# huawei-noah/xingtian

Hardware: NVIDIA H100
Metric: learner env-steps/sec (Atari 84x84x4 PPO) (higher is better)
Workload: dtype f32 (bf16x3 split on wgmma, fp32 accumulate in registers)

## Files before the change

xingtian_b200/csrc/bp_gemm.cuh:

```cuda
#pragma once
#include <cuda_bf16.h>
#include <cuda_runtime.h>
#include <stdint.h>

#include "gemm_f32.cuh"

#ifndef XTB_BP_WAIT_HINT
#define XTB_BP_WAIT_HINT 20000u
#endif

namespace xtb {
namespace bp {

typedef __nv_bfloat16 bf16;

__device__ __forceinline__ uint32_t smem_u32(const void* p) { return (uint32_t)__cvta_generic_to_shared(p); }
__device__ __forceinline__ void mbar_init(uint32_t bar, uint32_t count) {
  asm volatile("mbarrier.init.shared::cta.b64 [%0], %1;" ::"r"(bar), "r"(count) : "memory");
}
__device__ __forceinline__ void fence_barrier_init() { asm volatile("fence.mbarrier_init.release.cluster;" ::: "memory"); }
__device__ __forceinline__ void mbar_arrive(uint32_t bar) {
  asm volatile("mbarrier.arrive.shared::cta.b64 _, [%0];" ::"r"(bar) : "memory");
}
__device__ __forceinline__ void mbar_expect_tx(uint32_t bar, uint32_t bytes) {
// ... 180 lines not shown
  split2(v[6], v[7], hi.w, lo.w);
}

struct BpT {
  bf16* hi;
  long long lo_off;
  int pitch;
};
__host__ __device__ inline long long bp_index(int pitch, int row, int f) { return ((long long)(f >> 3) * pitch + row) * 8 + (f & 7); }

constexpr int BP_CONSUMER_WGS = 2;
constexpr int BP_P_WARP = 4 * BP_CONSUMER_WGS;
constexpr int BP_THREADS = 32 * (BP_P_WARP + 1);
constexpr int BP_CONSUMER_WARPS = 4 * BP_CONSUMER_WGS;

constexpr int RW_THREADS = BP_THREADS;
constexpr int RW_A_PLANE = 2048;
constexpr int RW_STAGE_A = 2 * 8 * RW_A_PLANE;
constexpr int RW_STAGE_B = 16384;
constexpr int RW_MAX_STAGES = 4;
constexpr int RW_EPI_BANKS = 2;

__host__ __device__ inline int dgrad_epi_planes(int src_act, int accumulate) {
  return (src_act == 1 ? 1 : (src_act == 2 ? 2 : 0)) + (accumulate ? 2 : 0);
}

struct StageEnt {
  uint32_t a_chunk;
  uint16_t w_row;
  uint16_t nch;
};
typedef uint32_t UnitEnt;
struct StageDesc { uint32_t a_off, w_off, nch; };

struct RowsArgs {
  BpT a; int a_split;
  const bf16* w_hi; const bf16* w_lo; int w_pitch;
  int w_res; int w_res_chunks;
  int mode;
  const StageEnt* stages; const UnitEnt* units;
  int n_stage_ents;
  int kchunks, kc_split, n_ntiles;
  int n_units, n_btiles, B, N;
  BpT out; float* out_f32; int ld_f32; const float* bias; float alpha; int act;
  float* part; long long part_z; int ld_part;
  BpT src; int src_act; int accumulate; float* db_part;
};

struct TileWalk {
  const uint2* stages_sm; const uint32_t* units_sm;
  uint32_t a_pstride, w_pitch; int mode, n_ntiles, kc_split, kchunks, N;
  const uint2* st; uint32_t a0, w0, da, dw; int ns, nch_last;
  __device__ __forceinline__ void setup(const RowsArgs& a, const uint2* s_sm, const uint32_t* u_sm) {
    stages_sm = s_sm; units_sm = u_sm;
    a_pstride = (uint32_t)a.a.pitch * 16u; w_pitch = (uint32_t)a.w_pitch;
    mode = a.mode; n_ntiles = a.n_ntiles; kc_split = a.kc_split; kchunks = a.kchunks; N = a.N;
  }
  template <int KIND>
// ... 11 lines not shown
      const uint32_t ue = units_sm[u];
      st = stages_sm + (ue & 0xffffffu); ns = (int)(ue >> 24);
    }
  }
  __device__ __forceinline__ StageDesc get(int s) const {
    if (st) {
      const uint2 v = st[s];
      return StageDesc{v.x * a_pstride, (v.y & 0xffffu) * 16u, v.y >> 16};
    }
    return StageDesc{a0 + (uint32_t)s * da, w0 + (uint32_t)s * dw, (uint32_t)(s == ns - 1 ? nch_last : 8)};
  }
};

template <int KIND, int N>
__global__ void __launch_bounds__(RW_THREADS, 1)
bp_rows_kernel(const __grid_constant__ RowsArgs a, int n_stages, int stage_bytes, int wres_bytes, int epi_banks) {
  extern __shared__ uint8_t smem_raw[];
  uint8_t* smem = reinterpret_cast<uint8_t*>((reinterpret_cast<uintptr_t>(smem_raw) + 127) & ~(uintptr_t)127);
  constexpr int NCH = N >> 3;
  const int epi_planes = KIND == 2 ? dgrad_epi_planes(a.src_act, a.accumulate) : 0;
  const int epi_bank_bytes = epi_planes * NCH * RW_A_PLANE;
  uint8_t* epi_sm = smem + wres_bytes + n_stages * stage_bytes;
  uint2* stages_sm = reinterpret_cast<uint2*>(epi_sm + epi_banks * epi_bank_bytes);
  uint32_t* units_sm = reinterpret_cast<uint32_t*>(stages_sm + a.n_stage_ents);
  __shared__ __align__(8) uint64_t bars[2 * RW_MAX_STAGES + 1 + 2 * RW_EPI_BANKS];
  __shared__ float red_sh[BP_CONSUMER_WARPS][64];
  __shared__ float bias_sh[64];

  const int tid = threadIdx.x, warp = __shfl_sync(0xffffffffu, tid >> 5, 0), lane = tid & 31;
  const uint32_t full0 = smem_u32(&bars[0]), empty0 = smem_u32(&bars[RW_MAX_STAGES]), wbar = smem_u32(&bars[2 * RW_MAX_STAGES]);
  const uint32_t efull0 = wbar + 8, eempty0 = efull0 + 8 * RW_EPI_BANKS;
  if (tid == 0) {
    for (int s = 0; s < RW_MAX_STAGES; s++) { mbar_init(full0 + 8 * s, 1); mbar_init(empty0 + 8 * s, BP_CONSUMER_WARPS); }
    mbar_init(wbar, 1);
    for (int k = 0; k < RW_EPI_BANKS; k++) { mbar_init(efull0 + 8 * k, 1); mbar_init(eempty0 + 8 * k, BP_CONSUMER_WARPS); }
    fence_barrier_init();
  }
  __syncthreads();
  if (a.mode != 2) {
    const uint2* gs = reinterpret_cast<const uint2*>(a.stages);
    for (int i = tid; i < a.n_stage_ents; i += RW_THREADS) stages_sm[i] = __ldg(gs + i);
    for (int i = tid; i < a.n_units; i += RW_THREADS) units_sm[i] = __ldg(a.units + i);
  }
  if (warp == BP_P_WARP && a.w_res && elect_one()) {
    const uint32_t bytes = (uint32_t)a.w_res_chunks * a.w_pitch * 16;
    mbar_expect_tx(wbar, 2 * bytes);
    bulk_g2s(smem_u32(smem), a.w_hi, bytes, wbar);
    bulk_g2s(smem_u32(smem) + bytes, a.w_lo, bytes, wbar);
  }
  pdl_wait();
  pdl_trigger();
  if (KIND == 0 && a.mode != 2 && tid < N) bias_sh[tid] = a.bias[tid];
  __syncthreads();
  const uint32_t wres = smem_u32(smem);
  const uint32_t stage0 = wres + (uint32_t)wres_bytes;
  const int total = a.n_units * a.n_btiles;
  constexpr bool CAT = (KIND != 2);
  const int nbt = a.n_btiles;
  const int du = (int)gridDim.x / nbt, dbt = (int)gridDim.x - du * nbt;

  if (warp == BP_P_WARP) {
    const bool a_split = a.a_split != 0, w_res = a.w_res != 0;
    const uint32_t a_pstride = (uint32_t)a.a.pitch * 16u, w_pstride = (uint32_t)a.w_pitch * 16u;
    const char* a_hi = reinterpret_cast<const char*>(a.a.hi);
    const char* a_lo = a_hi + a.a.lo_off * 2;
    const char* w_hi = reinterpret_cast<const char*>(a.w_hi);
    const char* w_lo = reinterpret_cast<const char*>(a.w_lo);
    constexpr int n_bh_fwd = N >> 3;
    int stage = 0; uint32_t phase = 0;
    int u = (int)blockIdx.x / nbt, bt = (int)blockIdx.x - u * nbt;
    const int Bsz = a.B;
    TileWalk tw; tw.setup(a, stages_sm, units_sm);
    const int src_act = a.src_act, accumulate = a.accumulate;
    const char* s_hi = reinterpret_cast<const char*>(a.src.hi);
    const char* s_lo = s_hi + a.src.lo_off * 2;
    const char* o_hi = reinterpret_cast<const char*>(a.out.hi);
    const char* o_lo = o_hi + a.out.lo_off * 2;
    const uint32_t s_ps = (uint32_t)a.src.pitch * 16u, o_ps = (uint32_t)a.out.pitch * 16u;
    int ebank = 0; uint32_t ephase = 0;
    for (int tile = blockIdx.x; tile < total; tile += gridDim.x) {
      const int b0 = bt * 128, nr = min(128, Bsz - b0);
      const uint32_t a_bytes = (uint32_t)nr * 16u, row_off = (uint32_t)b0 * 16u;
      tw.init<KIND>(u);
      for (int s = 0; s < tw.ns; s++) {
        const StageDesc d = tw.get(s);
        mbar_wait(empty0 + 8 * stage, phase ^ 1);
        const int nch = (int)d.nch;
        const int n_bh = w_res ? 0 : (KIND == 2 ? nch : n_bh_fwd);
        const uint32_t b_bytes = (KIND == 2) ? (uint32_t)N * 16u : (uint32_t)nch * 128u;
        const uint32_t fb = full0 + 8 * stage;
        if (elect_one()) {
          mbar_expect_tx(fb, a_bytes * (a_split ? 2 * nch : nch) + b_bytes * 2 * n_bh);
          const uint32_t sA = stage0 + (uint32_t)stage * stage_bytes, sB = sA + RW_STAGE_A;
          const char* ah = a_hi + d.a_off + row_off;
          for (int c = 0; c < nch; c++) bulk_g2s(sA + c * RW_A_PLANE, ah + (uint32_t)c * a_pstride, a_bytes, fb);
          if (a_split) {
            const char* al = a_lo + d.a_off + row_off;
            for (int c = 0; c < nch; c++) bulk_g2s(sA + 8 * RW_A_PLANE + c * RW_A_PLANE, al + (uint32_t)c * a_pstride, a_bytes, fb);
          }
          if (!w_res) {
            const char* wh = w_hi + d.w_off; const char* wl = w_lo + d.w_off;
            if (KIND == 2) {
              for (int c = 0; c < n_bh; c++) {
                bulk_g2s(sB + c * (N * 16), wh + (uint32_t)c * w_pstride, b_bytes, fb);
                bulk_g2s(sB + 8192 + c * (N * 16), wl + (uint32_t)c * w_pstride, b_bytes, fb);
              }
            } else {
              for (int c = 0; c < n_bh; c++) {
                bulk_g2s(sB + c * 1024, wh + (uint32_t)c * w_pstride, b_bytes, fb);
                bulk_g2s(sB + (n_bh_fwd + c) * 1024, wl + (uint32_t)c * w_pstride, b_bytes, fb);
              }
            }
          }
        }
        __syncwarp();
        if (++stage == n_stages) { stage = 0; phase ^= 1; }
      }
      if (KIND == 2 && epi_planes) {
        mbar_wait(eempty0 + 8 * ebank, ephase ^ 1);
        if (elect_one()) {
          const uint32_t fb = efull0 + 8 * ebank;
          mbar_expect_tx(fb, a_bytes * (uint32_t)(NCH * epi_planes));
          const uint32_t oc0 = (uint32_t)((tw.mode == 2 ? u % tw.n_ntiles : u) * NCH);
          uint32_t dst = smem_u32(epi_sm) + (uint32_t)(ebank * epi_bank_bytes);
          auto plane = [&](const char* base, uint32_t ps) {
            const char* src = base + oc0 * ps + row_off;
            for (int c = 0; c < NCH; c++, dst += RW_A_PLANE) bulk_g2s(dst, src + (uint32_t)c * ps, a_bytes, fb);
          };
          if (src_act == 1 || src_act == 2) plane(s_hi, s_ps);
          if (src_act == 2) plane(s_lo, s_ps);
          if (accumulate) { plane(o_hi, o_ps); plane(o_lo, o_ps); }
        }
        __syncwarp();
        if (++ebank == epi_banks) { ebank = 0; ephase ^= 1; }
      }
      u += du; bt += dbt;
      if (bt >= nbt) { bt -= nbt; u++; }
    }
  } else if (warp < BP_P_WARP) {
    constexpr int ACC = CAT ? 2 * N : N;
    float dbacc[N / 4];
#pragma unroll
    for (int j = 0; j < N / 4; j++) dbacc[j] = 0.f;
    const int wg = warp >> 2, q = lane & 3;
    const int row_in_tile = wg * 64 + (warp & 3) * 16 + (lane >> 2);
    const bool a_split = a.a_split != 0, w_res = a.w_res != 0;
    const int act = a.act, mode = a.mode, Bsz = a.B, n_nt = a.n_ntiles, ld_f32 = a.ld_f32, src_act = a.src_act, accumulate = a.accumulate;
    const int ld_part = a.ld_part;
    const float alpha = a.alpha;
    bf16* const out_hi = a.out.hi; const long long out_lo = a.out.lo_off;
    float* const out_f32 = a.out_f32; const float* const bias_g = a.bias;
    float* const part = a.part; const long long part_z = a.part_z;
    const long long out_pstride = (long long)a.out.pitch * 8;
    const int b_pad = (Bsz + 15) & ~15;
    const uint32_t epi_thr = smem_u32(epi_sm) + (uint32_t)(row_in_tile * 16 + 4 * q);
    const int epi_out_plane = epi_planes - (accumulate ? 2 : 0);
    int ebank = 0; uint32_t ephase = 0;
    const uint64_t adesc = make_desc(0, RW_A_PLANE, 128);
    const uint64_t bdesc = (KIND == 2) ? make_desc(0, (uint32_t)N * 16, 128) : make_desc(0, 128, 1024);
    const uint32_t a_row_add = (uint32_t)(wg * 64 * 16) >> 4;
    const uint32_t a_lo_add = (8 * RW_A_PLANE) >> 4, a_step = (2 * RW_A_PLANE) >> 4;
    const uint32_t w_pstride = (uint32_t)a.w_pitch * 16u;
    const uint64_t wdesc = (KIND == 2) ? make_desc(0, w_pstride, 128) : make_desc(0, 128, w_pstride);
    const uint32_t w_lo_add = ((uint32_t)a.w_res_chunks * w_pstride) >> 4;
    const uint32_t b_step = (KIND == 2) ? (w_res ? (2 * w_pstride) >> 4 : (2u * N * 16u) >> 4) : (256 >> 4);
    const uint32_t b_lo_add = w_res ? w_lo_add : (8192 >> 4);
    const uint64_t b_const = w_res ? wdesc : bdesc;
    if (w_res) mbar_wait(wbar, 0);
    int stage = 0; uint32_t phase = 0;
    int held = -1;
    auto idle = [&](int bt) { return bt * 128 + wg * 64 >= Bsz; };

    auto mma_stage = [&](float* acc, const StageDesc& d, bool first, bool skip) {
      mbar_wait(full0 + 8 * stage, phase);
      const uint32_t sA = stage0 + (uint32_t)stage * stage_bytes;
      uint32_t a_lo32 = (sA >> 4) + a_row_add;
      uint32_t b_lo32 = w_res ? (wres + d.w_off) >> 4 : (sA + RW_STAGE_A) >> 4;
      const int ksteps = __shfl_sync(0xffffffffu, skip ? 0 : (int)d.nch >> 1, 0);
      uint32_t sd = first ? 0u : 1u;
      wgmma_fence();
      if (a_split) {
        for (int j = 0; j < ksteps; j++) {
          const uint64_t ah = adesc | a_lo32, bh = b_const | b_lo32, al = adesc | (a_lo32 + a_lo_add);
          if (KIND != 2) {
            wgmma<2 * N, 0, 1>(acc, ah, bh, sd);
            wgmma<N, 0, 1>(acc, al, bh);
          } else {
            wgmma<N, 0, 0>(acc, ah, bh, sd);
            wgmma<N, 0, 0>(acc, ah, b_const | (b_lo32 + b_lo_add));
            wgmma<N, 0, 0>(acc, al, bh);
          }
          a_lo32 += a_step; b_lo32 += b_step; sd = 1u;
        }
      } else {
        for (int j = 0; j < ksteps; j++) {
          const uint64_t ah = adesc | a_lo32, bh = b_const | b_lo32;
          if (KIND != 2) {
            wgmma<2 * N, 0, 1>(acc, ah, bh, sd);
          } else {
            wgmma<N, 0, 0>(acc, ah, bh, sd);
            wgmma<N, 0, 0>(acc, ah, b_const | (b_lo32 + b_lo_add));
          }
          a_lo32 += a_step; b_lo32 += b_step; sd = 1u;
        }
      }
      wgmma_commit();
      wgmma_wait<1>();
      if (held >= 0 && lane == 0) mbar_arrive(empty0 + 8 * held);
      held = stage;
      if (++stage == n_stages) { stage = 0; phase ^= 1; }
    };

    int tile = blockIdx.x;
    int u = (int)blockIdx.x / nbt, bt = (int)blockIdx.x - u * nbt;
    TileWalk tw; tw.setup(a, stages_sm, units_sm);
    auto start_tile = [&](float* acc) {
      tw.init<KIND>(u);
      tw.ns = __shfl_sync(0xffffffffu, tw.ns, 0);
      if (tw.ns == 0) return false;
      discard_regs<ACC / 2>(acc);
      mma_stage(acc, tw.get(0), true, idle(bt));
      return true;
    };

    auto epilogue = [&](const float* cur, int cu, int cbt, bool empty, uint32_t eb) {
      const int btile0 = cbt * 128;
      int oc0, z = 0;
      if (mode == 2) { const int nt = cu % n_nt; z = cu / n_nt; oc0 = nt * NCH; }
      else oc0 = cu * NCH;
#pragma unroll
      for (int h = 0; h < 2; h++) {
        const int b = btile0 + row_in_tile + 8 * h;
#pragma unroll
        for (int i = 0; i < NCH; i++) {
          const int c = 8 * i + 2 * q;
          float v0 = cur[4 * i + 2 * h], v1 = cur[4 * i + 2 * h + 1];
          if (CAT) { v0 += cur[4 * (i + NCH) + 2 * h]; v1 += cur[4 * (i + NCH) + 2 * h + 1]; }
          if (empty) { v0 = 0.f; v1 = 0.f; }
          if (KIND == 0) {
            if (b < Bsz) {
              const int f = oc0 * 8 + c;
              float bb0, bb1;
              if (mode == 2) { const float2 t2 = __ldg(reinterpret_cast<const float2*>(bias_g + f)); bb0 = t2.x; bb1 = t2.y; }
              else { bb0 = bias_sh[c]; bb1 = bias_sh[c + 1]; }
              if (act == 2) { v0 = tanhf(alpha * v0 + bb0); v1 = tanhf(alpha * v1 + bb1); }
              else {
                const float lo = act == 1 ? 0.f : -INFINITY;
// ... 2 lines not shown
              if (out_hi) {
                bf16* p = out_hi + (long long)(oc0 + i) * out_pstride + (long long)b * 8 + 2 * q;
                uint32_t hi, lo;
                split2(v0, v1, hi, lo);
                *reinterpret_cast<uint32_t*>(p) = hi;
                *reinterpret_cast<uint32_t*>(p + out_lo) = lo;
              }
              if (out_f32) *reinterpret_cast<float2*>(out_f32 + (long long)b * ld_f32 + f) = make_float2(v0, v1);
            }
          } else if (KIND == 1) {
            if (b < Bsz)
              *reinterpret_cast<float2*>(part + (long long)z * part_z + (long long)b * ld_part + oc0 * 8 + c) = make_float2(v0, v1);
          } else {
            bf16* p = out_hi + (long long)(oc0 + i) * out_pstride + (long long)b * 8 + 2 * q;
            if (b < Bsz) {
              const uint32_t e = eb + (uint32_t)(i * RW_A_PLANE + 128 * h);
              if (src_act == 1) {
                float s0, s1;
                unpack2(lds_u32(e), s0, s1);
                v0 = s0 > 0.f ? v0 : 0.f; v1 = s1 > 0.f ? v1 : 0.f;
              } else if (src_act == 2) {
                float s0, s1, t0, t1;
                unpack2(lds_u32(e), s0, s1);
                unpack2(lds_u32(e + NCH * RW_A_PLANE), t0, t1);
                const float y0 = s0 + t0, y1 = s1 + t1;
                v0 *= 1.f - y0 * y0; v1 *= 1.f - y1 * y1;
              }
              dbacc[2 * i] += v0; dbacc[2 * i + 1] += v1;
              if (accumulate) {
                const uint32_t eo = e + (uint32_t)(epi_out_plane * NCH * RW_A_PLANE);
                float s0, s1, t0, t1;
                unpack2(lds_u32(eo), s0, s1);
                unpack2(lds_u32(eo + NCH * RW_A_PLANE), t0, t1);
                v0 += s0 + t0; v1 += s1 + t1;
              }
              uint32_t hi, lo;
              split2(v0, v1, hi, lo);
              *reinterpret_cast<uint32_t*>(p) = hi;
              *reinterpret_cast<uint32_t*>(p + out_lo) = lo;
            } else if (b < b_pad && !accumulate) {
              *reinterpret_cast<uint32_t*>(p) = 0u;
              *reinterpret_cast<uint32_t*>(p + out_lo) = 0u;
            }
          }
        }
      }
    };

    constexpr bool OVERLAP = !(KIND == 0 && N == 64);
    auto finish_tile = [&](float* cur, float* nxt) {
      for (int s = 1; s < tw.ns; s++) mma_stage(cur, tw.get(s), false, idle(bt));
      const bool empty = tw.ns == 0;
      const int cu = u, cbt = bt;
      tile += gridDim.x; u += du; bt += dbt;
      if (bt >= nbt) { bt -= nbt; u++; }
      if (!(OVERLAP && tile < total && start_tile(nxt))) {
        wgmma_wait<0>();
        if (held >= 0 && lane == 0) mbar_arrive(empty0 + 8 * held);
        held = -1;
      }
      fence_regs<ACC / 2>(cur);
      if (KIND == 2 && epi_planes) mbar_wait(efull0 + 8 * ebank, ephase);
      if (!idle(cbt)) epilogue(cur, cu, cbt, empty, epi_thr + (uint32_t)(ebank * epi_bank_bytes));
      if (KIND == 2 && epi_planes) {
        __syncwarp();
        if (lane == 0) mbar_arrive(eempty0 + 8 * ebank);
        if (++ebank == epi_banks) { ebank = 0; ephase ^= 1; }
      }
      if (!OVERLAP && tile < total) start_tile(nxt);
    };
    float acc0[ACC / 2], acc1[ACC / 2];
    if (tile < total) start_tile(acc0);
    while (tile < total) {
      finish_tile(acc0, acc1);
      if (tile >= total) break;
      finish_tile(acc1, acc0);
    }
    if (KIND == 2 && a.db_part) {
#pragma unroll
      for (int j = 0; j < N / 4; j++) {
        float s = dbacc[j];
        s += __shfl_xor_sync(0xffffffffu, s, 4);
        s += __shfl_xor_sync(0xffffffffu, s, 8);
        s += __shfl_xor_sync(0xffffffffu, s, 16);
        if (lane < 4) red_sh[warp][8 * (j >> 1) + 2 * lane + (j & 1)] = s;
      }
      asm volatile("bar.sync 1, %0;" ::"n"(32 * BP_CONSUMER_WARPS) : "memory");
      if (tid < N) {
        float t = 0.f;
#pragma unroll
        for (int w = 0; w < BP_CONSUMER_WARPS; w++) t += red_sh[w][tid];
// ... 454 lines not shown
```

xingtian_b200/csrc/xtb_engine.cu:

```cuda
#include "../../include/xtb200.h"

#include <cuda_runtime.h>

#include <atomic>
#include <cmath>
#include <cstdarg>
#include <cstdio>
#include <cstring>
#include <map>
#include <memory>
#include <string>
#include <tuple>
#include <vector>

#include "gemm_f32.cuh"
#include "optim.cuh"
#include "rl_kernels.cuh"
#include "per.cuh"
#include "muzero_replay.cuh"
#include "qmix.cuh"
#include "scc.cuh"
#include "infoflow.cuh"
#include "stager.cuh"
#include "bp_gemm.cuh"
// ... 263 lines not shown
static inline uint8_t forms(const xtb_net* n, int t, bool grad) { return grad ? n->cur[t].grad : n->cur[t].val; }
static inline void wrote(xtb_net* n, int t, bool grad, Form f) { (grad ? n->cur[t].grad : n->cur[t].val) = f; }
static void invalidate(xtb_net* n, bool values, bool grads) {
  for (TensorForms& c : n->cur) { if (values) c.val = kNone; if (grads) c.grad = kNone; }
}
static inline const bp::bf16* blob_hi(const xtb_net* n, const LayerPlan& lp) { return (const bp::bf16*)(n->ws + n->blob_off) + lp.blob_off; }
static inline bool use_tc(const LayerPlan& lp) { return g_tc_mode && lp.tc; }
struct ConvTabs { const int *koff, *kyx, *dkyx, *dco, *wk; };
static inline ConvTabs conv_tabs(const xtb_net* n, const LayerPlan& lp) {
  const int* t = (const int*)(n->ws + lp.im2col_off);
  return ConvTabs{t, t + lp.K, t + 2 * lp.K, t + 2 * lp.K + lp.Kd, t + 2 * lp.K + 2 * lp.Kd};
}

static int pick_tile(int n) { return n % 64 == 0 ? 64 : (n % 32 == 0 ? 32 : (n % 16 == 0 ? 16 : 0)); }

struct RowsSmem { int wres_bytes, stage_bytes, epi_bank_bytes, epi_banks, tab_bytes, n_stages; };
static RowsSmem rows_smem(bool w_res, int w_res_chunks, int w_pitch, int mode, size_t n_stage_ents, size_t n_units, int N,
                          int epi_planes) {
  RowsSmem r;
  r.wres_bytes = w_res ? (int)align_up((size_t)2 * w_res_chunks * w_pitch * 16, 128) : 0;
  r.stage_bytes = bp::RW_STAGE_A + (w_res ? 0 : bp::RW_STAGE_B);
  r.epi_bank_bytes = epi_planes * (N / 8) * bp::RW_A_PLANE;
  const size_t tab = mode == 2 ? 0 : align_up(n_stage_ents * sizeof(bp::StageEnt) + n_units * sizeof(bp::UnitEnt), 128);
  r.tab_bytes = (int)std::min(tab, (size_t)kMaxDynSmem + 1);
  const int room = kMaxDynSmem - 128 - r.wres_bytes - r.tab_bytes;
  auto stages = [&](int banks) { return std::max(0, std::min(bp::RW_MAX_STAGES, (room - banks * r.epi_bank_bytes) / r.stage_bytes)); };
  r.epi_banks = epi_planes ? bp::RW_EPI_BANKS : 0;
  r.n_stages = stages(r.epi_banks);
  if (r.n_stages < 2 && r.epi_banks > 1) { r.epi_banks = 1; r.n_stages = stages(1); }
  return r;
}
static inline int dgrad_act(const LayerPlan& lp) { return act_is_ext(lp.src_act) ? 0 : lp.src_act; }
static RowsSmem conv_dgrad_smem(const LayerPlan& lp, bool accumulate) {
  return rows_smem(lp.w_res, lp.N / 8, lp.K, 1, lp.dg_st.size(), lp.dg_un.size(), lp.n_dg,
                   bp::dgrad_epi_planes(dgrad_act(lp), accumulate));
}
static size_t wgrad_smem(int mode, int n_opix, int R) {
  return 128 + bp::WG_STAGES * bp::WG_STAGE + (mode == 0 ? align_up((size_t)n_opix * R * sizeof(bp::WgEnt), 128) : 0);
}
static int dense_k_slices(int kchunks, int tiles, int* kc_split) {
  *kc_split = kchunks;
  if (tiles < kSMs && kchunks >= 32) {
    const int want = std::min(kSMs / tiles, kchunks / 8);
    if (want > 1) {
      *kc_split = ((kchunks + want - 1) / want + 7) / 8 * 8;
      return (kchunks + *kc_split - 1) / *kc_split;
    }
  }
  return 1;
}
// ... 254 lines not shown
extern "C" int xtb_net_layer_plan(const xtb_net* net, int layer, xtb_layer_plan* out) {
  if (!net || !out || layer < 0 || layer >= (int)net->L.size()) return fail(XTB_ERR_ARG, "xtb_net_layer_plan: bad argument");
  const LayerPlan& lp = net->L[layer];
  memset(out, 0, sizeof *out);
  out->kind = lp.d.kind;
  if (!lp.tc) return XTB_OK;
  out->tc = 1; out->s2d = lp.s2d; out->w_res = lp.w_res;
  out->n_fwd = lp.n_fwd; out->n_dg = lp.n_dg; out->R = lp.R;
  if (lp.d.kind == XTB_CONV) {
    out->fwd_stages = rows_smem(lp.w_res, lp.N / 8, lp.K, 0, lp.fwd_st.size(), lp.fwd_un.size(), lp.n_fwd, 0).n_stages;
    out->dg_stages = conv_dgrad_smem(lp, false).n_stages;
    for (bp::UnitEnt u : lp.dg_un) out->dg_empty_units += (u >> 24) == 0;
    out->k_slices = 1;
  } else {
    out->fwd_stages = rows_smem(false, 0, lp.K, 2, 0, 0, lp.n_fwd, 0).n_stages;
    out->dg_stages = rows_smem(false, 0, lp.K, 2, 0, 0, lp.n_dg, bp::dgrad_epi_planes(dgrad_act(lp), 0)).n_stages;
    int kc_split;
    out->k_slices = dense_k_slices(lp.K / 8, (lp.N / lp.n_fwd) * ((net->max_batch + 127) / 128), &kc_split);
  }
  return XTB_OK;
}

extern "C" int xtb_net_tensor_size(const xtb_net* net, int t) {
  if (!net || t < 0 || t >= (int)net->tsize.size()) return -1;
  return net->tsize[t];
}

extern "C" size_t xtb_net_workspace_bytes(const xtb_net* net) { return net ? net->ws_bytes : 0; }

static cudaError_t ensure_kernel_attrs();
extern "C" int xtb_net_sync_weights(xtb_net* net, void* stream);
// ... 51 lines not shown
      return;
    }
    launch_cfg<32, 32, 2, 2>(al, bl, ep, M, N, K, 1, st);
    return;
  }
  long long c = ctas(64, 64);
  if (c >= kSMs || split_ok) {
    if (split_ok) { ksplit = (int)((2 * kSMs + c - 1) / c); int mx = (K + 63) / 64; if (ksplit > mx) ksplit = mx; if (ksplit < 1) ksplit = 1; }
    launch_cfg<64, 64, 4, 4>(al, bl, ep, M, N, K, ksplit, st);
    return;
  }
  launch_cfg<32, 32, 2, 2>(al, bl, ep, M, N, K, 1, st);
}

template <int KIND>
static void (*const kRowsKernels[])(bp::RowsArgs, int, int, int, int) = {
    bp::bp_rows_kernel<KIND, 16>, bp::bp_rows_kernel<KIND, 32>, bp::bp_rows_kernel<KIND, 48>, bp::bp_rows_kernel<KIND, 64>};
static void (*const kWgradKernels[])(bp::WgradArgs) = {bp::bp_wgrad_kernel<16>, bp::bp_wgrad_kernel<32>,
                                                       bp::bp_wgrad_kernel<48>, bp::bp_wgrad_kernel<64>};
template <class F, size_t C>
static F by_width(F const (&tab)[C], int n) { return n > 0 && n % 16 == 0 && n / 16 <= (int)C ? tab[n / 16 - 1] : nullptr; }

template <class F> struct HeadsEnt { int kpl, amax; F kern; };
template <class LOSS>
static const HeadsEnt<void (*)(PpoHeadsArgs)> kHeadsKernels[] = {
    {2, 8, heads_kernel<LOSS, 2, 8>}, {8, 4, heads_kernel<LOSS, 8, 4>}, {8, 8, heads_kernel<LOSS, 8, 8>},
    {16, 4, heads_kernel<LOSS, 16, 4>}};
template <class DIST>
static const HeadsEnt<decltype(&infer_heads_kernel<DIST, 2, 8>)> kInferHeadsKernels[] = {
    {2, 8, infer_heads_kernel<DIST, 2, 8>}, {8, 4, infer_heads_kernel<DIST, 8, 4>}, {8, 8, infer_heads_kernel<DIST, 8, 8>},
    {16, 8, infer_heads_kernel<DIST, 16, 8>}};
// ... 19 lines not shown
  for (auto k : kWgradKernels) opt_in((const void*)k);
  for (const auto& h : kHeadsKernels<PpoLoss>) opt_in((const void*)h.kern);
  for (const auto& h : kHeadsKernels<DuelingTdLoss>) opt_in((const void*)h.kern);
  for (const auto& h : kHeadsKernels<PpoGaussLoss>) opt_in((const void*)h.kern);
  done = e == cudaSuccess;
  return e;
}

template <int KIND>
static cudaError_t launch_rows(bp::RowsArgs& a, cudaStream_t st) {
  const auto kern = by_width(kRowsKernels<KIND>, a.N);
  if (!kern) return cudaErrorInvalidValue;
  { cudaError_t e0 = ensure_kernel_attrs(); if (e0 != cudaSuccess) return e0; }
  const int epi_planes = KIND == 2 ? bp::dgrad_epi_planes(a.src_act, a.accumulate) : 0;
  const RowsSmem m = rows_smem(a.w_res != 0, a.w_res_chunks, a.w_pitch, a.mode, (size_t)a.n_stage_ents, (size_t)a.n_units, a.N,
                               epi_planes);
  if (m.n_stages < 2) return cudaErrorInvalidConfiguration;
  const int smem = 128 + m.wres_bytes + m.n_stages * m.stage_bytes + m.epi_banks * m.epi_bank_bytes + m.tab_bytes;
  const int total = a.n_units * a.n_btiles;
  const int grid = std::min(total, kSMs);
  XLAUNCH(kern, grid, bp::RW_THREADS, smem, st, a, m.n_stages, m.stage_bytes, m.wres_bytes, m.epi_banks);
  return cudaPeekAtLastError();
}

static cudaError_t launch_wgrad(const bp::WgradArgs& a, int grid, cudaStream_t st) {
  const auto kern = by_width(kWgradKernels, a.N);
  if (!kern) return cudaErrorInvalidValue;
  { cudaError_t e0 = ensure_kernel_attrs(); if (e0 != cudaSuccess) return e0; }
  const size_t smem = wgrad_smem(a.mode, a.n_opix, a.R);
  if (smem > (size_t)kMaxDynSmem) return cudaErrorInvalidConfiguration;
  XLAUNCH(kern, grid, bp::WG_THREADS, (int)smem, st, a);
  return cudaPeekAtLastError();
}

static void queue_reduction(xtb_net* net, const float* part, int n_slabs, long long slab, int count, long long dst_off,
                            float* dst_ptr = nullptr, const LayerPlan* conv = nullptr) {
// ... 5 lines not shown
    r.N = conv->N; r.C = conv->q.C; r.KW = conv->q.KW; r.mts = conv->mts; r.s2d_k4 = conv->s2d ? conv->k4 : 0;
    r.alpha = conv->d.src == 0 ? net->desc.scale : 1.f;
  }
  net->pending.push_back(r);
}

static cudaError_t tc_forward(xtb_net* net, int i, int B, int split_rows, bool want_f32, bool want_bp, cudaStream_t st,
                              long long* launches) {
  const LayerPlan& lp = net->L[i];
  const int t = i + 1;
  bp::RowsArgs a;
  memset(&a, 0, sizeof a);
  a.a = lp.d.src == 0 ? obs_bp(net) : out_bp(net, lp.d.src);
  a.a_split = lp.d.src != 0;
  a.w_hi = blob_hi(net, lp); a.w_lo = a.w_hi + net->blob_elems; a.w_pitch = lp.K;
  a.B = B; a.n_btiles = (B + 127) / 128; a.N = lp.n_fwd;
  const bool ext = act_is_ext(lp.d.act);
  a.out = want_bp && !ext ? out_bp(net, t) : no_bp();
  a.out_f32 = ext ? pre_buf(net, t) : (want_f32 ? out_f32(net, t) : nullptr);
  a.ld_f32 = net->tsize[t];
  a.bias = net->params + lp.b_off;
  a.alpha = lp.d.src == 0 ? net->desc.scale : 1.f;
  a.act = ext ? 0 : lp.d.act;
  *launches = 1;
  if (lp.d.kind == XTB_CONV) {
    a.mode = 0;
    a.stages = (const bp::StageEnt*)(net->ws + lp.fwd_st_off); a.units = (const bp::UnitEnt*)(net->ws + lp.fwd_un_off);
    a.n_stage_ents = (int)lp.fwd_st.size();
    a.w_res = lp.w_res; a.w_res_chunks = lp.N / 8;
    a.n_units = lp.q.OH * lp.q.OW;
    return launch_rows<0>(a, st);
// ... 12 lines not shown
  if (e != cudaSuccess) return e;
  long long pieces = (long long)(lp.N / 8) * b_pad * bp::FIN_ZL;
  XLAUNCH(bp::bp_splitk_finish_kernel, (unsigned)((pieces + 127) / 128), 128, 0, st, (const float*)a.part, nz, a.part_z, B, lp.N,
          a.bias, a.act, a.out_f32, a.out);
  *launches = 2;
  return cudaPeekAtLastError();
}

static cudaError_t tc_dgrad(xtb_net* net, int i, int B, int accumulate, float* db_part, cudaStream_t st) {
  const LayerPlan& lp = net->L[i];
  const int t = i + 1, s = lp.d.src;
  bp::RowsArgs a;
  memset(&a, 0, sizeof a);
  a.a = gout_bp(net, t); a.a_split = 1;
  a.w_hi = blob_hi(net, lp); a.w_lo = a.w_hi + net->blob_elems; a.w_pitch = lp.K;
  a.B = B; a.n_btiles = (B + 127) / 128; a.N = lp.n_dg;
  a.out = gout_bp(net, s); a.src = out_bp(net, s); a.src_act = dgrad_act(lp); a.accumulate = accumulate; a.db_part = db_part;
  if (lp.d.kind == XTB_CONV) {
    a.mode = 1;
    a.stages = (const bp::StageEnt*)(net->ws + lp.dg_st_off); a.units = (const bp::UnitEnt*)(net->ws + lp.dg_un_off);
    a.n_stage_ents = (int)lp.dg_st.size();
    a.w_res = lp.w_res; a.w_res_chunks = lp.N / 8;
    a.n_units = lp.q.H * lp.q.W;
  } else {
    a.mode = 2;
    a.kchunks = lp.N / 8; a.kc_split = a.kchunks; a.n_ntiles = lp.K / lp.n_dg;
    a.n_units = a.n_ntiles;
  }
  return launch_rows<2>(a, st);
}

// ... 84 lines not shown
                                                        {&bias, std::max(N, 64)}, {&part, nz > 1 ? (long long)nz * M * N : 0}}))
    return rc;
  bp::BpT ta{pa, ea, pitch}, tw{pw, ew, mode == 2 ? pitch : K}, tcp{pc, ec, pitch};
  auto split = [&](const float* src, int B_, int F_, bp::BpT dst) {
    long long pieces = (long long)(F_ / 8) * ((B_ + 15) & ~15);
    XLAUNCH(bp::bp_split_kernel, (unsigned)((pieces + 127) / 128), 128, 0, st, src, B_, F_, dst);
  };
  cudaError_t e = cudaSuccess;
  if (mode == 0 || mode == 1) {
    split(a, M, K, ta);
    if (mode == 0) { tw.pitch = K; split(b, K, N, tw); }
    else { tw.pitch = (N + 15) / 16 * 16; split(b, N, K, tw); }
    bp::RowsArgs r;
    memset(&r, 0, sizeof r);
    r.a = ta; r.a_split = 1; r.w_hi = pw; r.w_lo = pw + ew; r.w_pitch = tw.pitch;
    r.mode = 2; r.B = M; r.n_btiles = (M + 127) / 128; r.N = nt; r.n_ntiles = N / nt;
    r.kchunks = kchunks; r.kc_split = kc_split;
    r.bias = bias; r.alpha = 1.f; r.act = 0;
    if (mode == 0) {
      r.n_units = r.n_ntiles * nz;
      if (nz > 1) {
        r.part = part; r.part_z = (long long)M * N; r.ld_part = N;
        e = launch_rows<1>(r, st);
        long long pieces = (long long)(N / 8) * ((M + 15) & ~15) * bp::FIN_ZL;
        XLAUNCH(bp::bp_splitk_finish_kernel, (unsigned)((pieces + 127) / 128), 128, 0, st, (const float*)part, nz, r.part_z, M, N,
                (const float*)bias, 0, c, no_bp());
      } else {
        r.out_f32 = c; r.ld_f32 = N;
        e = launch_rows<0>(r, st);
      }
    } else {
// ... 227 lines not shown
    LAUNCH_CHECK();
    wrote(net, s, true, kF32); wrote(net, s2, true, kF32);
    return XTB_OK;
  }
  if (use_tc(lp)) {
    int rc = ensure_bp(net, t, B, true, st);
    if (rc) return rc;
    if (dgrad_act(lp) != 0) { rc = ensure_bp(net, s, B, false, st); if (rc) return rc; }
    if (acc) { rc = ensure_bp(net, s, B, true, st); if (rc) return rc; }
    float* dbp = fuse_db ? (float*)(net->ws + lp.dbpart_off) : nullptr;
    cudaError_t te = tc_dgrad(net, i, B, acc, dbp, st);
    if (te != cudaSuccess) return fail(XTB_ERR_CUDA, "tensor-core dgrad launch (layer %d): %s", i, cudaGetErrorString(te));
    LAUNCH_CHECK();
    if (fuse_db) {
      const int units = lp.d.kind == XTB_CONV ? lp.q.H * lp.q.W : lp.K / lp.n_dg;
      queue_reduction(net, dbp, std::min(kSMs, units * ((B + 127) / 128)), lp.n_dg, lp.n_dg, net->L[s - 1].b_off);
    }
    wrote(net, s, true, kPlanes);
    return XTB_OK;
  }
  int rc = ensure_f32(net, t, B, true, st);
  if (rc) return rc;
  rc = ensure_f32(net, s, B, false, st);
  if (rc) return rc;
  if (acc) { rc = ensure_f32(net, s, B, true, st); if (rc) return rc; }
  const float* dy = gout_f32(net, t);
  const float* x = out_f32(net, s);
  float* gsrc = gout_f32(net, s);
  const float* w = net->params + lp.w_off;
  if (lp.d.kind == XTB_CONV) {
    const ConvTabs tab = conv_tabs(net, lp);
// ... 2362 lines not shown
```

Before: 286,100.

## Split rows kernel into independent per-warpgroup rings with 64-row work items

The rows GEMM kernel can now run each consumer warpgroup as its own pipeline ring, with its own producer warp, stage buffers, mbarriers and epilogue banks, working on 64-row slices instead of shared 128-row tiles. The host picks between the old paired layout (128 rows) and independent rings based on shared-memory stage capacity, and falls back to paired tiles when bias partial sums are fused. This aims to cut load imbalance and idle warpgroups at small or ragged batch sizes and to let the two warpgroups progress independently. The cost is an extra producer warp, duplicated weight-tile loads per ring when weights are not resident, and possibly fewer pipeline stages per ring.

```diff
diff --git a/xingtian_b200/csrc/bp_gemm.cuh b/xingtian_b200/csrc/bp_gemm.cuh
--- a/xingtian_b200/csrc/bp_gemm.cuh
+++ b/xingtian_b200/csrc/bp_gemm.cuh
@@ -218,8 +218,9 @@
 constexpr int BP_THREADS = 32 * (BP_P_WARP + 1);
 constexpr int BP_CONSUMER_WARPS = 4 * BP_CONSUMER_WGS;
 
-constexpr int RW_THREADS = BP_THREADS;
-constexpr int RW_A_PLANE = 2048;
+constexpr int RW_THREADS = 32 * (BP_P_WARP + BP_CONSUMER_WGS);
+constexpr int RW_ROWS = 64;
+constexpr int RW_A_PLANE = RW_ROWS * 16;
 constexpr int RW_STAGE_A = 2 * 8 * RW_A_PLANE;
 constexpr int RW_STAGE_B = 16384;
 constexpr int RW_MAX_STAGES = 4;
@@ -245,7 +246,7 @@
   const StageEnt* stages; const UnitEnt* units;
   int n_stage_ents;
   int kchunks, kc_split, n_ntiles;
-  int n_units, n_btiles, B, N;
+  int n_units, n_slices, B, N;
   BpT out; float* out_f32; int ld_f32; const float* bias; float alpha; int act;
   float* part; long long part_z; int ld_part;
   BpT src; int src_act; int accumulate; float* db_part;
@@ -287,26 +288,35 @@
 
 template <int KIND, int N>
 __global__ void __launch_bounds__(RW_THREADS, 1)
-bp_rows_kernel(const __grid_constant__ RowsArgs a, int n_stages, int stage_bytes, int wres_bytes, int epi_banks) {
+bp_rows_kernel(const __grid_constant__ RowsArgs a, int n_stages, int stage_bytes, int wres_bytes, int epi_banks, int item_wgs) {
   extern __shared__ uint8_t smem_raw[];
   uint8_t* smem = reinterpret_cast<uint8_t*>((reinterpret_cast<uintptr_t>(smem_raw) + 127) & ~(uintptr_t)127);
   constexpr int NCH = N >> 3;
+  const int rings = BP_CONSUMER_WGS / item_wgs, rows = RW_ROWS * item_wgs;
+  const int a_plane = rows * 16;
   const int epi_planes = KIND == 2 ? dgrad_epi_planes(a.src_act, a.accumulate) : 0;
-  const int epi_bank_bytes = epi_planes * NCH * RW_A_PLANE;
-  uint8_t* epi_sm = smem + wres_bytes + n_stages * stage_bytes;
-  uint2* stages_sm = reinterpret_cast<uint2*>(epi_sm + epi_banks * epi_bank_bytes);
+  const int epi_bank_bytes = epi_planes * NCH * a_plane;
+  uint8_t* epi_sm = smem + wres_bytes + rings * n_stages * stage_bytes;
+  uint2* stages_sm = reinterpret_cast<uint2*>(epi_sm + rings * epi_banks * epi_bank_bytes);
   uint32_t* units_sm = reinterpret_cast<uint32_t*>(stages_sm + a.n_stage_ents);
-  __shared__ __align__(8) uint64_t bars[2 * RW_MAX_STAGES + 1 + 2 * RW_EPI_BANKS];
+  constexpr int WG_BARS = 2 * RW_MAX_STAGES + 2 * RW_EPI_BANKS;
+  __shared__ __align__(8) uint64_t bars[BP_CONSUMER_WGS * WG_BARS + 1];
   __shared__ float red_sh[BP_CONSUMER_WARPS][64];
   __shared__ float bias_sh[64];
 
   const int tid = threadIdx.x, warp = __shfl_sync(0xffffffffu, tid >> 5, 0), lane = tid & 31;
-  const uint32_t full0 = smem_u32(&bars[0]), empty0 = smem_u32(&bars[RW_MAX_STAGES]), wbar = smem_u32(&bars[2 * RW_MAX_STAGES]);
-  const uint32_t efull0 = wbar + 8, eempty0 = efull0 + 8 * RW_EPI_BANKS;
+  const uint32_t wbar = smem_u32(&bars[BP_CONSUMER_WGS * WG_BARS]);
   if (tid == 0) {
-    for (int s = 0; s < RW_MAX_STAGES; s++) { mbar_init(full0 + 8 * s, 1); mbar_init(empty0 + 8 * s, BP_CONSUMER_WARPS); }
+    const uint32_t readers = 4 * item_wgs;
+    for (int g = 0; g < rings; g++) {
+      const uint32_t b0 = smem_u32(&bars[g * WG_BARS]);
+      for (int s = 0; s < RW_MAX_STAGES; s++) { mbar_init(b0 + 8 * s, 1); mbar_init(b0 + 8 * (RW_MAX_STAGES + s), readers); }
+      for (int k = 0; k < RW_EPI_BANKS; k++) {
+        mbar_init(b0 + 8 * (2 * RW_MAX_STAGES + k), 1);
+        mbar_init(b0 + 8 * (2 * RW_MAX_STAGES + RW_EPI_BANKS + k), readers);
+      }
+    }
     mbar_init(wbar, 1);
-    for (int k = 0; k < RW_EPI_BANKS; k++) { mbar_init(efull0 + 8 * k, 1); mbar_init(eempty0 + 8 * k, BP_CONSUMER_WARPS); }
     fence_barrier_init();
   }
   __syncthreads();
@@ -326,13 +336,21 @@
   if (KIND == 0 && a.mode != 2 && tid < N) bias_sh[tid] = a.bias[tid];
   __syncthreads();
   const uint32_t wres = smem_u32(smem);
-  const uint32_t stage0 = wres + (uint32_t)wres_bytes;
-  const int total = a.n_units * a.n_btiles;
+  const int n_units = a.n_units;
   constexpr bool CAT = (KIND != 2);
-  const int nbt = a.n_btiles;
-  const int du = (int)gridDim.x / nbt, dbt = (int)gridDim.x - du * nbt;
-
-  if (warp == BP_P_WARP) {
+  const int nsl = a.n_slices;
+  const int step = rings * (int)gridDim.x;
+  const int du = step / nsl, dsl = step - du * nsl;
+  const int ring = warp < BP_P_WARP ? (warp >> 2) / item_wgs : warp - BP_P_WARP;
+  const int first = rings * (int)blockIdx.x + ring;
+  const uint32_t full0 = smem_u32(&bars[ring * WG_BARS]), empty0 = full0 + 8 * RW_MAX_STAGES;
+  const uint32_t efull0 = empty0 + 8 * RW_MAX_STAGES, eempty0 = efull0 + 8 * RW_EPI_BANKS;
+  const uint32_t stage0 = wres + (uint32_t)wres_bytes + (uint32_t)(ring * n_stages * stage_bytes);
+  const uint32_t epi0 = smem_u32(epi_sm) + (uint32_t)(ring * epi_banks * epi_bank_bytes);
+  const uint32_t stage_a = 16u * (uint32_t)a_plane;
+
+  if (warp >= BP_P_WARP) {
+    if (ring >= rings) return;
     const bool a_split = a.a_split != 0, w_res = a.w_res != 0;
     const uint32_t a_pstride = (uint32_t)a.a.pitch * 16u, w_pstride = (uint32_t)a.w_pitch * 16u;
     const char* a_hi = reinterpret_cast<const char*>(a.a.hi);
@@ -341,7 +359,7 @@
     const char* w_lo = reinterpret_cast<const char*>(a.w_lo);
     constexpr int n_bh_fwd = N >> 3;
     int stage = 0; uint32_t phase = 0;
-    int u = (int)blockIdx.x / nbt, bt = (int)blockIdx.x - u * nbt;
+    int u = first / nsl, sl = first - u * nsl;
     const int Bsz = a.B;
     TileWalk tw; tw.setup(a, stages_sm, units_sm);
     const int src_act = a.src_act, accumulate = a.accumulate;
@@ -351,8 +369,8 @@
     const char* o_lo = o_hi + a.out.lo_off * 2;
     const uint32_t s_ps = (uint32_t)a.src.pitch * 16u, o_ps = (uint32_t)a.out.pitch * 16u;
     int ebank = 0; uint32_t ephase = 0;
-    for (int tile = blockIdx.x; tile < total; tile += gridDim.x) {
-      const int b0 = bt * 128, nr = min(128, Bsz - b0);
+    while (u < n_units) {
+      const int b0 = sl * rows, nr = min(rows, Bsz - b0);
       const uint32_t a_bytes = (uint32_t)nr * 16u, row_off = (uint32_t)b0 * 16u;
       tw.init<KIND>(u);
       for (int s = 0; s < tw.ns; s++) {
@@ -364,12 +382,12 @@
         const uint32_t fb = full0 + 8 * stage;
         if (elect_one()) {
           mbar_expect_tx(fb, a_bytes * (a_split ? 2 * nch : nch) + b_bytes * 2 * n_bh);
-          const uint32_t sA = stage0 + (uint32_t)stage * stage_bytes, sB = sA + RW_STAGE_A;
+          const uint32_t sA = stage0 + (uint32_t)stage * stage_bytes, sB = sA + stage_a;
           const char* ah = a_hi + d.a_off + row_off;
-          for (int c = 0; c < nch; c++) bulk_g2s(sA + c * RW_A_PLANE, ah + (uint32_t)c * a_pstride, a_bytes, fb);
+          for (int c = 0; c < nch; c++) bulk_g2s(sA + c * a_plane, ah + (uint32_t)c * a_pstride, a_bytes, fb);
           if (a_split) {
             const char* al = a_lo + d.a_off + row_off;
-            for (int c = 0; c < nch; c++) bulk_g2s(sA + 8 * RW_A_PLANE + c * RW_A_PLANE, al + (uint32_t)c * a_pstride, a_bytes, fb);
+            for (int c = 0; c < nch; c++) bulk_g2s(sA + (8 + c) * a_plane, al + (uint32_t)c * a_pstride, a_bytes, fb);
           }
           if (!w_res) {
             const char* wh = w_hi + d.w_off; const char* wl = w_lo + d.w_off;
@@ -395,10 +413,10 @@
           const uint32_t fb = efull0 + 8 * ebank;
           mbar_expect_tx(fb, a_bytes * (uint32_t)(NCH * epi_planes));
           const uint32_t oc0 = (uint32_t)((tw.mode == 2 ? u % tw.n_ntiles : u) * NCH);
-          uint32_t dst = smem_u32(epi_sm) + (uint32_t)(ebank * epi_bank_bytes);
+          uint32_t dst = epi0 + (uint32_t)(ebank * epi_bank_bytes);
           auto plane = [&](const char* base, uint32_t ps) {
             const char* src = base + oc0 * ps + row_off;
-            for (int c = 0; c < NCH; c++, dst += RW_A_PLANE) bulk_g2s(dst, src + (uint32_t)c * ps, a_bytes, fb);
+            for (int c = 0; c < NCH; c++, dst += a_plane) bulk_g2s(dst, src + (uint32_t)c * ps, a_bytes, fb);
           };
           if (src_act == 1 || src_act == 2) plane(s_hi, s_ps);
           if (src_act == 2) plane(s_lo, s_ps);
@@ -407,16 +425,17 @@
         __syncwarp();
         if (++ebank == epi_banks) { ebank = 0; ephase ^= 1; }
       }
-      u += du; bt += dbt;
-      if (bt >= nbt) { bt -= nbt; u++; }
-    }
-  } else if (warp < BP_P_WARP) {
+      u += du; sl += dsl;
+      if (sl >= nsl) { sl -= nsl; u++; }
+    }
+  } else {
     constexpr int ACC = CAT ? 2 * N : N;
     float dbacc[N / 4];
 #pragma unroll
     for (int j = 0; j < N / 4; j++) dbacc[j] = 0.f;
-    const int wg = warp >> 2, q = lane & 3;
-    const int row_in_tile = wg * 64 + (warp & 3) * 16 + (lane >> 2);
+    const int q = lane & 3;
+    const int wg_row0 = ((warp >> 2) % item_wgs) * RW_ROWS;
+    const int row_in_item = wg_row0 + (warp & 3) * 16 + (lane >> 2);
     const bool a_split = a.a_split != 0, w_res = a.w_res != 0;
     const int act = a.act, mode = a.mode, Bsz = a.B, n_nt = a.n_ntiles, ld_f32 = a.ld_f32, src_act = a.src_act, accumulate = a.accumulate;
     const int ld_part = a.ld_part;
@@ -426,13 +445,13 @@
     float* const part = a.part; const long long part_z = a.part_z;
     const long long out_pstride = (long long)a.out.pitch * 8;
     const int b_pad = (Bsz + 15) & ~15;
-    const uint32_t epi_thr = smem_u32(epi_sm) + (uint32_t)(row_in_tile * 16 + 4 * q);
+    const uint32_t epi_thr = epi0 + (uint32_t)(row_in_item * 16 + 4 * q);
     const int epi_out_plane = epi_planes - (accumulate ? 2 : 0);
     int ebank = 0; uint32_t ephase = 0;
-    const uint64_t adesc = make_desc(0, RW_A_PLANE, 128);
+    const uint64_t adesc = make_desc(0, 0, 128);
     const uint64_t bdesc = (KIND == 2) ? make_desc(0, (uint32_t)N * 16, 128) : make_desc(0, 128, 1024);
-    const uint32_t a_row_add = (uint32_t)(wg * 64 * 16) >> 4;
-    const uint32_t a_lo_add = (8 * RW_A_PLANE) >> 4, a_step = (2 * RW_A_PLANE) >> 4;
+    const uint32_t a_add = (uint32_t)make_desc((uint32_t)(wg_row0 * 16), (uint32_t)a_plane, 0);
+    const uint32_t a_step = (uint32_t)(2 * a_plane) >> 4;
     const uint32_t w_pstride = (uint32_t)a.w_pitch * 16u;
     const uint64_t wdesc = (KIND == 2) ? make_desc(0, w_pstride, 128) : make_desc(0, 128, w_pstride);
     const uint32_t w_lo_add = ((uint32_t)a.w_res_chunks * w_pstride) >> 4;
@@ -442,19 +461,20 @@
     if (w_res) mbar_wait(wbar, 0);
     int stage = 0; uint32_t phase = 0;
     int held = -1;
-    auto idle = [&](int bt) { return bt * 128 + wg * 64 >= Bsz; };
+    const int idle_sl = (Bsz - wg_row0 + rows - 1) / rows;
+    auto idle = [&](int sl) { return KIND == 2 && sl >= idle_sl; };
 
     auto mma_stage = [&](float* acc, const StageDesc& d, bool first, bool skip) {
       mbar_wait(full0 + 8 * stage, phase);
       const uint32_t sA = stage0 + (uint32_t)stage * stage_bytes;
-      uint32_t a_lo32 = (sA >> 4) + a_row_add;
-      uint32_t b_lo32 = w_res ? (wres + d.w_off) >> 4 : (sA + RW_STAGE_A) >> 4;
+      uint32_t a_lo32 = a_add + (sA >> 4);
+      uint32_t b_lo32 = w_res ? (wres + d.w_off) >> 4 : (sA >> 4) + 8 * a_step;
       const int ksteps = __shfl_sync(0xffffffffu, skip ? 0 : (int)d.nch >> 1, 0);
       uint32_t sd = first ? 0u : 1u;
       wgmma_fence();
       if (a_split) {
         for (int j = 0; j < ksteps; j++) {
-          const uint64_t ah = adesc | a_lo32, bh = b_const | b_lo32, al = adesc | (a_lo32 + a_lo_add);
+          const uint64_t ah = adesc | a_lo32, bh = b_const | b_lo32, al = adesc | (a_lo32 + 4 * a_step);
           if (KIND != 2) {
             wgmma<2 * N, 0, 1>(acc, ah, bh, sd);
             wgmma<N, 0, 1>(acc, al, bh);
@@ -484,26 +504,25 @@
       if (++stage == n_stages) { stage = 0; phase ^= 1; }
     };
 
-    int tile = blockIdx.x;
-    int u = (int)blockIdx.x / nbt, bt = (int)blockIdx.x - u * nbt;
+    int u = first / nsl, sl = first - u * nsl;
     TileWalk tw; tw.setup(a, stages_sm, units_sm);
-    auto start_tile = [&](float* acc) {
+    auto start_item = [&](float* acc) {
       tw.init<KIND>(u);
       tw.ns = __shfl_sync(0xffffffffu, tw.ns, 0);
       if (tw.ns == 0) return false;
       discard_regs<ACC / 2>(acc);
-      mma_stage(acc, tw.get(0), true, idle(bt));
+      mma_stage(acc, tw.get(0), true, idle(sl));
       return true;
     };
 
-    auto epilogue = [&](const float* cur, int cu, int cbt, bool empty, uint32_t eb) {
-      const int btile0 = cbt * 128;
+    auto epilogue = [&](const float* cur, int cu, int csl, bool empty, uint32_t eb) {
+      const int brow0 = csl * (int)(a_step >> 1);
       int oc0, z = 0;
       if (mode == 2) { const int nt = cu % n_nt; z = cu / n_nt; oc0 = nt * NCH; }
       else oc0 = cu * NCH;
 #pragma unroll
       for (int h = 0; h < 2; h++) {
-        const int b = btile0 + row_in_tile + 8 * h;
+        const int b = brow0 + row_in_item + 8 * h;
 #pragma unroll
         for (int i = 0; i < NCH; i++) {
           const int c = 8 * i + 2 * q;
@@ -536,7 +555,7 @@
           } else {
             bf16* p = out_hi + (long long)(oc0 + i) * out_pstride + (long long)b * 8 + 2 * q;
             if (b < Bsz) {
-              const uint32_t e = eb + (uint32_t)(i * RW_A_PLANE + 128 * h);
+              const uint32_t e = eb + (uint32_t)(i * a_plane + 128 * h);
               if (src_act == 1) {
                 float s0, s1;
                 unpack2(lds_u32(e), s0, s1);
@@ -544,16 +563,16 @@
               } else if (src_act == 2) {
                 float s0, s1, t0, t1;
                 unpack2(lds_u32(e), s0, s1);
-                unpack2(lds_u32(e + NCH * RW_A_PLANE), t0, t1);
+                unpack2(lds_u32(e + NCH * a_plane), t0, t1);
                 const float y0 = s0 + t0, y1 = s1 + t1;
                 v0 *= 1.f - y0 * y0; v1 *= 1.f - y1 * y1;
               }
               dbacc[2 * i] += v0; dbacc[2 * i + 1] += v1;
               if (accumulate) {
-                const uint32_t eo = e + (uint32_t)(epi_out_plane * NCH * RW_A_PLANE);
+                const uint32_t eo = e + (uint32_t)(epi_out_plane * NCH * a_plane);
                 float s0, s1, t0, t1;
                 unpack2(lds_u32(eo), s0, s1);
-                unpack2(lds_u32(eo + NCH * RW_A_PLANE), t0, t1);
+                unpack2(lds_u32(eo + NCH * a_plane), t0, t1);
                 v0 += s0 + t0; v1 += s1 + t1;
               }
               uint32_t hi, lo;
@@ -570,33 +589,33 @@
     };
 
     constexpr bool OVERLAP = !(KIND == 0 && N == 64);
-    auto finish_tile = [&](float* cur, float* nxt) {
-      for (int s = 1; s < tw.ns; s++) mma_stage(cur, tw.get(s), false, idle(bt));
+    auto finish_item = [&](float* cur, float* nxt) {
+      for (int s = 1; s < tw.ns; s++) mma_stage(cur, tw.get(s), false, idle(sl));
       const bool empty = tw.ns == 0;
-      const int cu = u, cbt = bt;
-      tile += gridDim.x; u += du; bt += dbt;
-      if (bt >= nbt) { bt -= nbt; u++; }
-      if (!(OVERLAP && tile < total && start_tile(nxt))) {
+      const int cu = u, csl = sl;
+      u += du; sl += dsl;
+      if (sl >= nsl) { sl -= nsl; u++; }
+      if (!(OVERLAP && u < n_units && start_item(nxt))) {
         wgmma_wait<0>();
         if (held >= 0 && lane == 0) mbar_arrive(empty0 + 8 * held);
         held = -1;
       }
       fence_regs<ACC / 2>(cur);
       if (KIND == 2 && epi_planes) mbar_wait(efull0 + 8 * ebank, ephase);
-      if (!idle(cbt)) epilogue(cur, cu, cbt, empty, epi_thr + (uint32_t)(ebank * epi_bank_bytes));
+      if (!idle(csl)) epilogue(cur, cu, csl, empty, epi_thr + (uint32_t)(ebank * epi_bank_bytes));
       if (KIND == 2 && epi_planes) {
         __syncwarp();
         if (lane == 0) mbar_arrive(eempty0 + 8 * ebank);
         if (++ebank == epi_banks) { ebank = 0; ephase ^= 1; }
       }
-      if (!OVERLAP && tile < total) start_tile(nxt);
+      if (!OVERLAP && u < n_units) start_item(nxt);
     };
     float acc0[ACC / 2], acc1[ACC / 2];
-    if (tile < total) start_tile(acc0);
-    while (tile < total) {
-      finish_tile(acc0, acc1);
-      if (tile >= total) break;
-      finish_tile(acc1, acc0);
+    if (u < n_units) start_item(acc0);
+    while (u < n_units) {
+      finish_item(acc0, acc1);
+      if (u >= n_units) break;
+      finish_item(acc1, acc0);
     }
     if (KIND == 2 && a.db_part) {
 #pragma unroll
diff --git a/xingtian_b200/csrc/xtb_engine.cu b/xingtian_b200/csrc/xtb_engine.cu
--- a/xingtian_b200/csrc/xtb_engine.cu
+++ b/xingtian_b200/csrc/xtb_engine.cu
@@ -301,26 +301,45 @@
 
 static int pick_tile(int n) { return n % 64 == 0 ? 64 : (n % 32 == 0 ? 32 : (n % 16 == 0 ? 16 : 0)); }
 
-struct RowsSmem { int wres_bytes, stage_bytes, epi_bank_bytes, epi_banks, tab_bytes, n_stages; };
-static RowsSmem rows_smem(bool w_res, int w_res_chunks, int w_pitch, int mode, size_t n_stage_ents, size_t n_units, int N,
-                          int epi_planes) {
+struct RowsSmem {
+  int wres_bytes, stage_bytes, epi_bank_bytes, epi_banks, tab_bytes, n_stages, item_wgs;
+  int rings() const { return bp::BP_CONSUMER_WGS / item_wgs; }
+  int bytes() const { return 128 + wres_bytes + rings() * (n_stages * stage_bytes + epi_banks * epi_bank_bytes) + tab_bytes; }
+};
+static RowsSmem rows_smem_for(int item_wgs, bool w_res, int w_res_chunks, int w_pitch, int mode, size_t n_stage_ents,
+                              size_t n_units, int N, int epi_planes) {
   RowsSmem r;
+  r.item_wgs = item_wgs;
   r.wres_bytes = w_res ? (int)align_up((size_t)2 * w_res_chunks * w_pitch * 16, 128) : 0;
-  r.stage_bytes = bp::RW_STAGE_A + (w_res ? 0 : bp::RW_STAGE_B);
-  r.epi_bank_bytes = epi_planes * (N / 8) * bp::RW_A_PLANE;
+  r.stage_bytes = item_wgs * bp::RW_STAGE_A + (w_res ? 0 : bp::RW_STAGE_B);
+  r.epi_bank_bytes = epi_planes * (N / 8) * item_wgs * bp::RW_A_PLANE;
   const size_t tab = mode == 2 ? 0 : align_up(n_stage_ents * sizeof(bp::StageEnt) + n_units * sizeof(bp::UnitEnt), 128);
   r.tab_bytes = (int)std::min(tab, (size_t)kMaxDynSmem + 1);
-  const int room = kMaxDynSmem - 128 - r.wres_bytes - r.tab_bytes;
-  auto stages = [&](int banks) { return std::max(0, std::min(bp::RW_MAX_STAGES, (room - banks * r.epi_bank_bytes) / r.stage_bytes)); };
+  const int room = kMaxDynSmem - 128 - r.wres_bytes - r.tab_bytes, R = r.rings();
+  auto stages = [&](int banks) { return std::max(0, std::min(bp::RW_MAX_STAGES, (room - R * banks * r.epi_bank_bytes) / (R * r.stage_bytes))); };
   r.epi_banks = epi_planes ? bp::RW_EPI_BANKS : 0;
   r.n_stages = stages(r.epi_banks);
   if (r.n_stages < 2 && r.epi_banks > 1) { r.epi_banks = 1; r.n_stages = stages(1); }
   return r;
 }
+static RowsSmem rows_smem(bool w_res, int w_res_chunks, int w_pitch, int mode, size_t n_stage_ents, size_t n_units, int N,
+                          int epi_planes, bool bias_sums = false) {
+  const RowsSmem tiles = rows_smem_for(2, w_res, w_res_chunks, w_pitch, mode, n_stage_ents, n_units, N, epi_planes);
+  if (bias_sums) return tiles;
+  const RowsSmem items = rows_smem_for(1, w_res, w_res_chunks, w_pitch, mode, n_stage_ents, n_units, N, epi_planes);
+  return items.n_stages >= tiles.n_stages && items.epi_banks >= tiles.epi_banks ? items : tiles;
+}
+static int rows_slices(const RowsSmem& m, int B) { const int rows = m.item_wgs * bp::RW_ROWS; return (B + rows - 1) / rows; }
+static int rows_grid(const RowsSmem& m, int n_units, int B) {
+  return (int)std::min<long long>(((long long)n_units * rows_slices(m, B) + m.rings() - 1) / m.rings(), kSMs);
+}
 static inline int dgrad_act(const LayerPlan& lp) { return act_is_ext(lp.src_act) ? 0 : lp.src_act; }
-static RowsSmem conv_dgrad_smem(const LayerPlan& lp, bool accumulate) {
+static RowsSmem conv_dgrad_smem(const LayerPlan& lp, bool accumulate, bool bias_sums = false) {
   return rows_smem(lp.w_res, lp.N / 8, lp.K, 1, lp.dg_st.size(), lp.dg_un.size(), lp.n_dg,
-                   bp::dgrad_epi_planes(dgrad_act(lp), accumulate));
+                   bp::dgrad_epi_planes(dgrad_act(lp), accumulate), bias_sums);
+}
+static RowsSmem dense_dgrad_smem(const LayerPlan& lp, bool accumulate, bool bias_sums = false) {
+  return rows_smem(false, 0, lp.K, 2, 0, 0, lp.n_dg, bp::dgrad_epi_planes(dgrad_act(lp), accumulate), bias_sums);
 }
 static size_t wgrad_smem(int mode, int n_opix, int R) {
   return 128 + bp::WG_STAGES * bp::WG_STAGE + (mode == 0 ? align_up((size_t)n_opix * R * sizeof(bp::WgEnt), 128) : 0);
@@ -605,7 +624,7 @@
     out->k_slices = 1;
   } else {
     out->fwd_stages = rows_smem(false, 0, lp.K, 2, 0, 0, lp.n_fwd, 0).n_stages;
-    out->dg_stages = rows_smem(false, 0, lp.K, 2, 0, 0, lp.n_dg, bp::dgrad_epi_planes(dgrad_act(lp), 0)).n_stages;
+    out->dg_stages = dense_dgrad_smem(lp, false).n_stages;
     int kc_split;
     out->k_slices = dense_k_slices(lp.K / 8, (lp.N / lp.n_fwd) * ((net->max_batch + 127) / 128), &kc_split);
   }
@@ -687,7 +706,7 @@
 }
 
 template <int KIND>
-static void (*const kRowsKernels[])(bp::RowsArgs, int, int, int, int) = {
+static void (*const kRowsKernels[])(bp::RowsArgs, int, int, int, int, int) = {
     bp::bp_rows_kernel<KIND, 16>, bp::bp_rows_kernel<KIND, 32>, bp::bp_rows_kernel<KIND, 48>, bp::bp_rows_kernel<KIND, 64>};
 static void (*const kWgradKernels[])(bp::WgradArgs) = {bp::bp_wgrad_kernel<16>, bp::bp_wgrad_kernel<32>,
                                                        bp::bp_wgrad_kernel<48>, bp::bp_wgrad_kernel<64>};
@@ -737,12 +756,11 @@
   { cudaError_t e0 = ensure_kernel_attrs(); if (e0 != cudaSuccess) return e0; }
   const int epi_planes = KIND == 2 ? bp::dgrad_epi_planes(a.src_act, a.accumulate) : 0;
   const RowsSmem m = rows_smem(a.w_res != 0, a.w_res_chunks, a.w_pitch, a.mode, (size_t)a.n_stage_ents, (size_t)a.n_units, a.N,
-                               epi_planes);
+                               epi_planes, KIND == 2 && a.db_part);
   if (m.n_stages < 2) return cudaErrorInvalidConfiguration;
-  const int smem = 128 + m.wres_bytes + m.n_stages * m.stage_bytes + m.epi_banks * m.epi_bank_bytes + m.tab_bytes;
-  const int total = a.n_units * a.n_btiles;
-  const int grid = std::min(total, kSMs);
-  XLAUNCH(kern, grid, bp::RW_THREADS, smem, st, a, m.n_stages, m.stage_bytes, m.wres_bytes, m.epi_banks);
+  a.n_slices = rows_slices(m, a.B);
+  XLAUNCH(kern, rows_grid(m, a.n_units, a.B), bp::RW_THREADS, m.bytes(), st, a, m.n_stages, m.stage_bytes, m.wres_bytes,
+          m.epi_banks, m.item_wgs);
   return cudaPeekAtLastError();
 }
 
@@ -778,7 +796,7 @@
   a.a = lp.d.src == 0 ? obs_bp(net) : out_bp(net, lp.d.src);
   a.a_split = lp.d.src != 0;
   a.w_hi = blob_hi(net, lp); a.w_lo = a.w_hi + net->blob_elems; a.w_pitch = lp.K;
-  a.B = B; a.n_btiles = (B + 127) / 128; a.N = lp.n_fwd;
+  a.B = B; a.N = lp.n_fwd;
   const bool ext = act_is_ext(lp.d.act);
   a.out = want_bp && !ext ? out_bp(net, t) : no_bp();
   a.out_f32 = ext ? pre_buf(net, t) : (want_f32 ? out_f32(net, t) : nullptr);
@@ -821,7 +839,7 @@
   memset(&a, 0, sizeof a);
   a.a = gout_bp(net, t); a.a_split = 1;
   a.w_hi = blob_hi(net, lp); a.w_lo = a.w_hi + net->blob_elems; a.w_pitch = lp.K;
-  a.B = B; a.n_btiles = (B + 127) / 128; a.N = lp.n_dg;
+  a.B = B; a.N = lp.n_dg;
   a.out = gout_bp(net, s); a.src = out_bp(net, s); a.src_act = dgrad_act(lp); a.accumulate = accumulate; a.db_part = db_part;
   if (lp.d.kind == XTB_CONV) {
     a.mode = 1;
@@ -936,7 +954,7 @@
     bp::RowsArgs r;
     memset(&r, 0, sizeof r);
     r.a = ta; r.a_split = 1; r.w_hi = pw; r.w_lo = pw + ew; r.w_pitch = tw.pitch;
-    r.mode = 2; r.B = M; r.n_btiles = (M + 127) / 128; r.N = nt; r.n_ntiles = N / nt;
+    r.mode = 2; r.B = M; r.N = nt; r.n_ntiles = N / nt;
     r.kchunks = kchunks; r.kc_split = kc_split;
     r.bias = bias; r.alpha = 1.f; r.act = 0;
     if (mode == 0) {
@@ -1194,7 +1212,8 @@
     LAUNCH_CHECK();
     if (fuse_db) {
       const int units = lp.d.kind == XTB_CONV ? lp.q.H * lp.q.W : lp.K / lp.n_dg;
-      queue_reduction(net, dbp, std::min(kSMs, units * ((B + 127) / 128)), lp.n_dg, lp.n_dg, net->L[s - 1].b_off);
+      const RowsSmem m = lp.d.kind == XTB_CONV ? conv_dgrad_smem(lp, acc, true) : dense_dgrad_smem(lp, acc, true);
+      queue_reduction(net, dbp, rows_grid(m, units, B), lp.n_dg, lp.n_dg, net->L[s - 1].b_off);
     }
     wrote(net, s, true, kPlanes);
     return XTB_OK;
```

After: 306,800 (median of 6 runs). +7.3%, better.
